# OettlM/STEDM

Measured on AMD Instinct MI355X. Metric: U-Net denoising steps/sec (32x32x4 latent, bs=64), higher is better.
Workload: dtype f16; 1 GPU; HER2-style DDIM-50 + CFG 1.5 (rescale 0.7) denoising step, NS32 U-Net (234.6M params, random-init PRNG weights), 32x32x4 latents + 3-ch layout concat, style vector 512; batch_per_gpu=64, global_batch=64, latent=32x32x4, cfg=cond+uncond per step, parallelism=dp1 (independent latents, no in-loop collective)

## Files before the change

### include/stedm_hip.h

```cpp
#ifndef STEDM_HIP_H
#define STEDM_HIP_H

#include <stdint.h>

#ifdef __cplusplus
extern "C" {
#endif

#define STEDM_ABI_VERSION 31

#define STEDM_F16 0
#define STEDM_BF16 1

#define STEDM_CONV_S1 0
#define STEDM_CONV_DOWN 1
#define STEDM_CONV_UP 2
#define STEDM_CONV_UP_SUBPIXEL 3
#define STEDM_CONV_S2D 4

int stedm_abi_version(void);
const char* stedm_last_error(void);
int stedm_device_cus(void);

#define STEDM_F16G_RAW 1
// ... 106 lines not shown
  float qkv_qscale;
  const float* ln_gamma;
  const float* ln_beta;
  const float* ln_res;
  float ln_eps;
  int32_t out16_stride;
  void* gn_coop;
  const uint32_t* gn_coop_epoch;
  uint32_t* gn_coop_tmo;
  int32_t src16_cstride;
  int32_t k_chan0;
  int32_t w_cin;
  int32_t res_bmod;
  const float* res2;
  int32_t ws_bmod;
} stedm_conv_args;
int stedm_conv_igemm(const stedm_conv_args* args, void* stream);
int stedm_conv_fused_skip_ok(const stedm_conv_args* args);
int stedm_conv3x3_tiles_ok(int Hout, int Wout);
int stedm_im2col_rows16(const void* src16, void* dst16, int B, int Hs, int Ws, int C, int mode, void* stream);
int stedm_conv_rs_ok(const stedm_conv_args* args);
int stedm_conv_partials(const stedm_conv_args* args, int32_t* nshare, int dry, void* stream);
int stedm_conv_finish(const stedm_conv_args* args, int nshare, void* stream);

int stedm_conv_in(const float* x1, int c1, const float* x2, int c2, int x2_bmod, const float* w_oihw,
                  const float* bias, float* out, int B, int H, int W, int cout, float* chan_stats, void* stream);
int stedm_conv_out(const float* src, int c, const float* chan_stats, int nslab, const float* gamma, const float* beta,
                   float eps, int groups, const float* w_hwio, const float* bias, float* out, int B, int H, int W,
                   int cout, void* stream);

// ... 226 lines not shown

int stedm_image_to_uint8(const float* x, unsigned char* out, int B, int C, int H, int W, void* stream);
int stedm_seg_merge(const float* seg, float* out, int B, int K, int H, int W, void* stream);
int stedm_argmax_u8(const float* seg, unsigned char* out, long N, int ncls, void* stream);

int stedm_unfold_tiles(const float* x, float* tiles, int B, int C, int H, int W, int kh, int kw, int sy, int sx, int l0, int nl, void* stream);
int stedm_fold_blend(const float* tiles, const float* w_tile, const float* w_tie, float* out, unsigned char* out_u8, int B, int C, int th, int tw,
                     int sy, int sx, int Ly, int Lx, void* stream);

int stedm_graph_begin(void* stream);
int stedm_graph_end(void* stream, void** graph_exec_out);
int stedm_graph_launch(void* graph_exec, void* stream);
int stedm_graph_destroy(void* graph_exec);

int stedm_debug_conv_stamps(unsigned long long* host_out, int nblocks);

#ifdef __cplusplus
}
#endif
#endif
```

### stedm_amd/_lib.py

```python
from __future__ import annotations

import ctypes as C
import os

_HERE = os.path.dirname(os.path.abspath(__file__))
LIB_PATH = os.environ.get("STEDM_HIP_LIB") or os.path.join(_HERE, "libstedm_hip.so")

ABI_VERSION = 31
F16, BF16 = 0, 1
CONV_S1, CONV_DOWN, CONV_UP, CONV_UP_SUBPIXEL, CONV_S2D = 0, 1, 2, 3, 4
STREAM_POSTERIOR = 0x40000


class StedmHipError(RuntimeError):
    pass


class ConvArgs(C.Structure):
    _fields_ = [
        ("src1", C.c_void_p), ("src2", C.c_void_p),
        ("c1", C.c_int32), ("c2", C.c_int32), ("src2_bmod", C.c_int32),
        ("B", C.c_int32), ("Hin", C.c_int32), ("Win", C.c_int32),
        ("mode", C.c_int32), ("ks", C.c_int32),
        ("scale", C.c_void_p), ("shift", C.c_void_p),
# ... 3 lines not shown
        ("res", C.c_void_p), ("out", C.c_void_p),
        ("cout", C.c_int32), ("npass", C.c_int32), ("mm_dtype", C.c_int32),
        ("src16_hi", C.c_void_p), ("src16_lo", C.c_void_p),
        ("act_out", C.c_int32), ("out16_hi", C.c_void_p), ("out16_lo", C.c_void_p),
        ("w_frag", C.c_void_p), ("chan_stats", C.c_void_p),
        ("src16b_hi", C.c_void_p), ("w_frag_b", C.c_void_p), ("bias_b", C.c_void_p), ("cb", C.c_int32),
        ("ws", C.c_void_p), ("ws_floats", C.c_int64), ("chan_nslab", C.c_int32), ("w_frag16", C.c_void_p), ("w_frag_b16", C.c_void_p), ("pad_br", C.c_int32),
        ("gn_gamma", C.c_void_p), ("gn_beta", C.c_void_p), ("gn_eps", C.c_float), ("gn_groups", C.c_int32), ("gn_act", C.c_int32), ("gn_out16", C.c_void_p), ("gn_mr", C.c_void_p), ("gn_only", C.c_int32),
        ("gn_out16_lo", C.c_void_p),
        ("qkv_q", C.c_void_p), ("qkv_k", C.c_void_p), ("qkv_vt", C.c_void_p),
        ("qkv_T", C.c_int32), ("qkv_Tp", C.c_int32), ("qkv_heads", C.c_int32), ("qkv_qscale", C.c_float),
        ("ln_gamma", C.c_void_p), ("ln_beta", C.c_void_p), ("ln_res", C.c_void_p), ("ln_eps", C.c_float),
        ("out16_stride", C.c_int32),
        ("gn_coop", C.c_void_p), ("gn_coop_epoch", C.c_void_p), ("gn_coop_tmo", C.c_void_p),
        ("src16_cstride", C.c_int32), ("k_chan0", C.c_int32), ("w_cin", C.c_int32), ("res_bmod", C.c_int32),
        ("res2", C.c_void_p), ("ws_bmod", C.c_int32),
    ]


_P, _I, _F = C.c_void_p, C.c_int, C.c_float
SIGNATURES = {
    "stedm_abi_version": (_I, []),
    "stedm_last_error": (C.c_char_p, []),
    "stedm_device_cus": (_I, []),
    "stedm_f16_guard_set": (_I, [_P]),
    "stedm_pack_conv_weight": (_I, [_P, _P, _P, _I, _I, _I, _I, _P]),
    "stedm_pack_conv_weight_up": (_I, [_P, _P, _P, _I, _I, _I, _P]),
    "stedm_pack_conv_weight_frag": (_I, [_P, _P, _I, _I, _I, _I, _P]),
    "stedm_pack_conv_weight_up_frag": (_I, [_P, _P, _I, _I, _I, _P]),
    "stedm_pack_conv_weight_frag16": (_I, [_P, C.c_long, C.c_long, _I, _P, _I, _I, _I, _I, _P]),
    "stedm_pack_conv_weight_frag16_hl": (_I, [_P, C.c_long, C.c_long, _I, _P, _I, _I, _I, _P]),
# ... 137 lines not shown
    "stedm_vq_nearest": (_I, [_P, _P, _I, _I, _I, C.c_long, _P, _P, _P]),
    "stedm_ddim_quantize_x0": (_I, [_P, _P, _P, _P, _P, _P, _I, _I, _I, C.c_long, _P, _P, _P]),
    "stedm_conv1x1_nchw": (_I, [_P, _P, _P, _P, _I, _I, _I, C.c_long, _P]),
    "stedm_softmax_rows16": (_I, [_P, C.c_long, _F, _P, _P, C.c_long, _I, C.c_long, _I, _P]),
    "stedm_gauss_sample": (_I, [_P, _P, _P, _I, _I, C.c_long, _F, _I, C.c_long, C.c_ulonglong, _P]),
    "stedm_image_to_uint8": (_I, [_P, _P, _I, _I, _I, _I, _P]),
    "stedm_seg_merge": (_I, [_P, _P, _I, _I, _I, _I, _P]),
    "stedm_argmax_u8": (_I, [_P, _P, C.c_long, _I, _P]),
    "stedm_unfold_tiles": (_I, [_P, _P, _I, _I, _I, _I, _I, _I, _I, _I, _I, _I, _P]),
    "stedm_fold_blend": (_I, [_P, _P, _P, _P, _P, _I, _I, _I, _I, _I, _I, _I, _I, _P]),
    "stedm_graph_begin": (_I, [_P]),
    "stedm_graph_end": (_I, [_P, C.POINTER(C.c_void_p)]),
    "stedm_graph_launch": (_I, [_P, _P]),
    "stedm_graph_destroy": (_I, [_P]),
    "stedm_debug_conv_stamps": (_I, [_P, _I]),
}

_lib = None


def lib() -> C.CDLL:
    global _lib
    if _lib is None:
        if not os.path.exists(LIB_PATH):
            raise StedmHipError(
                f"{LIB_PATH} not found: build it with `python -m stedm_amd.build` "
                "(there is no CPU / PyTorch fallback for the hot path)")
        try:
            import torch
        except ImportError:
# ... 24 lines not shown
```

### stedm_amd/csrc/conv_common.hpp

```cpp
#pragma once
#include "common.hpp"

typedef float f32x16 __attribute__((ext_vector_type(16)));
typedef float f32x4 __attribute__((ext_vector_type(4)));
typedef _Float16 f16x8 __attribute__((ext_vector_type(8)));
typedef __bf16 bf16x8 __attribute__((ext_vector_type(8)));
typedef _Float16 f16x4 __attribute__((ext_vector_type(4)));
typedef __bf16 bf16x4 __attribute__((ext_vector_type(4)));

constexpr int BN = 128;

struct ConvParams {
  stedm_conv_args a;
  int M, Hout, Wout, HWout, Cin, taps;
  int cstride, w_cin;
  int whole, nsamp, trows;
  int wsplit;
  int PRs, PW, NP;
  int tiles_m, tiles_n;
  unsigned mg_hw, mg_w, mg_pw, mg_prpw;
  int ksplit;
  int stats_done;
  int gn_done;
  int gn_tile;
  int gn_coop;
  int xcd_m;
  int partials;
  int nshare;
  int npers;
  unsigned* ovf;
  int dbg;
};

#ifdef STEDM_CONV_DIAG
#define STEDM_DBG(WORD, BITS) (((WORD) & (BITS)) != 0)
#else
#define STEDM_DBG(WORD, BITS) (0)
#endif

template <typename T>
struct MM;
template <>
struct MM<_Float16> {
  using V8 = f16x8;
  using V4 = f16x4;
  static __device__ __forceinline__ f32x16 mfma(V8 a, V8 b, f32x16 c) {
    return __builtin_amdgcn_mfma_f32_32x32x16_f16(a, b, c, 0, 0, 0);
  }
  static __device__ __forceinline__ f32x4 mfma16(V8 a, V8 b, f32x4 c) {
    return __builtin_amdgcn_mfma_f32_16x16x32_f16(a, b, c, 0, 0, 0);
  }
};
template <>
// ... 3 lines not shown
  static __device__ __forceinline__ f32x16 mfma(V8 a, V8 b, f32x16 c) {
    return __builtin_amdgcn_mfma_f32_32x32x16_bf16(a, b, c, 0, 0, 0);
  }
  static __device__ __forceinline__ f32x4 mfma16(V8 a, V8 b, f32x4 c) {
    return __builtin_amdgcn_mfma_f32_16x16x32_bf16(a, b, c, 0, 0, 0);
  }
};


#define STEDM_ZERO_PAGE_BYTES 135168

namespace stedm {
bool conv_geometry(ConvParams& p, int bm, bool allow_wsplit = false);
int conv_launch_dma(ConvParams& p, hipStream_t st, bool dry = false);
int conv_splitk_finish(ConvParams& p, int nshare, hipStream_t st);
}
```

### stedm_amd/csrc/conv_dma_bf16_p1.hip

```cpp
#include "conv_igemm_dma9.inc"
#include "conv_rs.inc"
namespace stedm {
int conv_dma_pick_bf16_p1(ConvParams& p, hipStream_t st, bool dry) {
  int rc = conv_rs_pick<__bf16>(p, st, dry);
  if (rc >= 0 || dry || p.a.src16b_hi || p.a.mode == STEDM_CONV_S2D || p.a.qkv_q || p.a.ln_gamma) return rc;
  if (p.a.src16_cstride || p.a.k_chan0 || p.a.w_cin || p.a.res_bmod || p.a.res2 || p.partials || p.a.out16_stride) return rc;
  rc = dma9_pick<__bf16>(p, st);
  return rc >= 0 ? rc : dma_pick<1, __bf16>(p, st);
}
}

extern "C" int stedm_debug_conv_stamps(unsigned long long* host_out, int nblocks) {
  if (!host_out || nblocks <= 0 || nblocks > 2048) { stedm::set_error("debug_conv_stamps: bad args"); return 1; }
  hipError_t e = hipMemcpyFromSymbol(host_out, HIP_SYMBOL(g_conv_stamps), (size_t)nblocks * 8 * sizeof(unsigned long long));
  if (e != hipSuccess) { stedm::set_error("debug_conv_stamps: %s", hipGetErrorString(e)); return 2; }
  return 0;
}
```

### stedm_amd/csrc/conv_igemm_dma.hip

```cpp
#include "conv_common.hpp"
using namespace stedm;

namespace stedm {
int conv_dma_pick_f16_p1(ConvParams&, hipStream_t, bool dry);
int conv_dma_pick_f16_p3(ConvParams&, hipStream_t, bool dry);
int conv_dma_pick_bf16_p1(ConvParams&, hipStream_t, bool dry);
int conv_dma_pick_bf16_p3(ConvParams&, hipStream_t, bool dry);
}

int stedm::conv_launch_dma(ConvParams& p, hipStream_t st, bool dry) {
  const stedm_conv_args& a = p.a;
  if (a.src16b_hi && a.npass != 1) { set_error("conv_igemm(dma): the fused skip phase is single-product only"); return 1; }
  if (dry && a.npass != 1 && !a.w_frag16) return 1;
  if (a.src16b_hi && ((long)a.B * a.Hin * a.Win * a.cb >= (1L << 31) || a.cb * 2 + 256 > STEDM_ZERO_PAGE_BYTES)) {
    set_error("conv_igemm(dma): fused skip operand too large (cb=%d)", a.cb);
    return 1;
  }
  if ((long)a.B * a.Hin * a.Win * (p.cstride > p.Cin ? p.cstride : p.Cin) >= (1L << 31)) {
    set_error("conv_igemm(dma): activation tensor too large for 32-bit element offsets");
    return 1;
  }
  if (p.Cin * 2 + 256 > STEDM_ZERO_PAGE_BYTES) { set_error("conv_igemm(dma): Cin too large for the zero page"); return 1; }
  const bool f16 = a.mm_dtype == STEDM_F16;
  int rc = a.npass == 3 ? (f16 ? conv_dma_pick_f16_p3(p, st, dry) : conv_dma_pick_bf16_p3(p, st, dry))
// ... 13 lines not shown
```

### stedm_amd/csrc/conv_rs.inc

```
#pragma once
#include <type_traits>

#include "conv_igemm_dma.inc"
#include "gn_fold.hpp"

static __device__ unsigned long long g_conv_stamps[2048 * 8];
#define STAMP(K) if (STEDM_DBG(p.dbg, 1024) && tid == 0 && blockIdx.x < 2048) g_conv_stamps[blockIdx.x * 8 + (K)] = wall_clock64()
#define STAMPC(K) if (STEDM_DBG(p.dbg, 1024) && tid == 0 && blockIdx.x < 2048) g_conv_stamps[blockIdx.x * 8 + (K)] = __builtin_amdgcn_s_memtime()

#ifdef STEDM_CONV_DIAG
#define RS_DIAG(BIT) ((STEDM_CONV_DIAG) & (BIT))
#else
#define RS_DIAG(BIT) 0
#endif

__device__ __forceinline__ float rs_lane_xor1(float v) {
  return __builtin_bit_cast(float, __builtin_amdgcn_mov_dpp(__builtin_bit_cast(int, v), 0xB1, 0xF, 0xF, true));
}
template <typename T>
__device__ __forceinline__ unsigned rs_pack2(float lo, float hi) {
  typedef T V2T __attribute__((ext_vector_type(2)));
  V2T v; v[0] = (T)lo; v[1] = (T)hi;
  return __builtin_bit_cast(unsigned, v);
}
// ... 28 lines not shown
    GLDB(bf[ST][0], sb_, 0); GLDB(bf[ST][1], sb_, 1024);                       \
  }
#define LOAD_A(BASE, SUB, ST)                                                  \
  {                                                                            \
    const unsigned pb_ = (BASE) + ((SUB) / NTAB) * a_plane;                    \
    _Pragma("unroll") for (int i_ = 0; i_ < WM; ++i_) { const unsigned a_ = pb_ + aofs[(SUB) % NTAB][i_]; LDSR(af[ST][i_], a_); } \
  }
#define LOAD_A1(BASE, SUB, ST, I)                                              \
  {                                                                            \
    const unsigned a_ = (BASE) + ((SUB) / NTAB) * a_plane + aofs[(SUB) % NTAB][I]; \
    LDSR(af[ST][I], a_);                                                       \
  }
#pragma unroll
  for (int k = 0; k < NSB; ++k) LOAD_B(k, k)
  if (FIRST) __syncthreads();
  {
    const unsigned Afirst = A0 + abuf * a_buf;
#pragma unroll
    for (int k = 0; k < LA; ++k) LOAD_A(Afirst, k, k)
  }
  if constexpr (!SPREAD) {
  for (int step = 0; step < nchunks; ++step) {
    const unsigned Acur = A0 + abuf * a_buf;
    if (++abuf == NABUF) abuf = 0;
    const unsigned Anext = step + 1 < nchunks ? A0 + abuf * a_buf : Acur;
    const int g0 = step * NS;
#pragma unroll
    for (int t = 0; t < NS; ++t) {
      if (!NOBAR && t == NS - LA - 1) __builtin_amdgcn_s_barrier();
      __builtin_amdgcn_sched_barrier(0);
#pragma unroll
      for (int j = 0; j < 2; ++j) acc[0][j] = RS_MFMA(af[t % NSA][0], bf[t % NSB][j], acc[0][j]);
      __builtin_amdgcn_sched_barrier(0);
      if (t + LA < NS) LOAD_A(Acur, t + LA, (t + LA) % NSA) else LOAD_A(Anext, t + LA - NS, (t + LA) % NSA)
      __builtin_amdgcn_sched_barrier(0);
// ... 62 lines not shown
    wcur = wsb + ((size_t)(unsigned)g_ << 13);                                 \
  }
#define W_LOAD(ST, C) if constexpr (!RS_DIAG(16)) bf[ST][C] = *reinterpret_cast<const V8*>(wcur + (C) * 1024);
#define A_ADDR(DST, BASE, TAP, HF, I)                                                                         \
  {                                                                                                           \
    if constexpr (NSETS == 1) asm volatile("v_add_u32 %0, %1, %2" : "=v"(DST) : "s"((BASE) + tapd[TAP]), "v"(aofs[0][(HF) * 4 + (I)])); \
    else asm volatile("v_add_u32 %0, %1, %2" : "=v"(DST) : "s"(BASE), "v"(aofs[NSETS == 1 ? 0 : (TAP)][(HF) * 4 + (I)]));           \
  }
#pragma unroll
  for (int k = 0; k < NSB; ++k) {
    W_ADDR(k)
#pragma unroll
    for (int c = 0; c < 4; ++c) W_LOAD(k, c)
  }
  if (FIRST) __syncthreads();
  {
    const unsigned Afirst = A0 + abuf * a_buf;
#pragma unroll
    for (int i = 0; i < 4; ++i) { unsigned a_; A_ADDR(a_, Afirst, 0, 0, i) if constexpr (!RS_DIAG(8)) LDSR(af[i], a_); }
  }
  for (int step = 0; step < nchunks; ++step) {
    const unsigned Acur = A0 + abuf * a_buf;
    if (++abuf == NABUF) abuf = 0;
    const unsigned Anext = step + 1 < nchunks ? A0 + abuf * a_buf : Acur;
    const int g0 = step * NS;
#pragma unroll
    for (int u = 0; u < NU; ++u) {
      const int t = u >> 1, hf = u & 1;
      if (u == NU - 1 && !RS_DIAG(32)) __builtin_amdgcn_s_barrier();
#pragma unroll
      for (int i = 0; i < 4; ++i) {
        const int pi = (i + 3) & 3;
        const int tu = i == 0 ? u : u + 1;
        unsigned a_ = 0;
#pragma unroll
// ... 178 lines not shown
    tile_n = (j - jm * tn_x) * gn + x / gm;
    tile_m = jm * gm + x % gm;
  }
  constexpr bool npers = NPERS;
  if (npers) { tile_m = bid / p.npers; tile_n = (bid % p.npers) * (p.tiles_n / p.npers); }
  if STEDM_DBG(p.dbg, 256) { tile_n = 0; tile_m = 0; }
  const int m0 = tile_m * BMT, n0 = tile_n * BN;
  const int nchunks_all = p.Cin / BKC;
  const int nchunks_w = p.w_cin / BKC;
  const int nsteps = split ? nchunks_all / p.ksplit : nchunks_all;
  const int cbeg = kz * nsteps;
  const int nsteps2_all = FUSE ? a.cb / 64 : 0;
  const int nsteps2 = split ? nsteps2_all / p.ksplit : nsteps2_all;
  const int c2beg = split ? kz * nsteps2 : 0;
  STAMP(0);

  int b0, yo0;
  if (p.whole) { b0 = tile_m * p.nsamp; yo0 = 0; }
  else { b0 = m0 / p.HWout; yo0 = (m0 - b0 * p.HWout) / p.Wout; }
  const int br = s2d ? a.pad_br : 0;
  const int x0 = p.wsplit ? (m0 - b0 * p.HWout) - yo0 * p.Wout : 0;
  const int srow0 = ((a.mode == STEDM_CONV_S1 || SUBPIX) ? yo0 - 1 : (yo0 - 1) >> 1) + br;
  static_assert(RS_3X3 == 0, "");

  auto div_hw = [&](int n) { return (int)__umulhi((unsigned)n, p.mg_hw); };
  auto div_w = [&](int n) { return (int)__umulhi((unsigned)n, p.mg_w); };
  auto div_pw = [&](int n) { return (int)__umulhi((unsigned)n, p.mg_pw); };
  auto div_prpw = [&](int n) { return (int)__umulhi((unsigned)n, p.mg_prpw); };
  const int rem0 = GEO1 ? m0 - (m0 / p.HWout) * p.HWout : 0;
  auto patch_pixel = [&](int pos) {
    int off = -1;
    if (pos < p.NP) {
      if (GEO1) { if (m0 + pos < p.M) off = m0 + pos; }
      else {
        const int s_ = div_prpw(pos), rem = pos - s_ * (p.PRs * p.PW);
        const int prow = div_pw(rem), pcol = rem - prow * p.PW;
        const int b = b0 + s_, sy = srow0 + prow, sx = x0 + pcol - 1 + br;
        if (b < a.B && sy >= 0 && sy < a.Hin && sx >= 0 && sx < a.Win) off = (b * a.Hin + sy) * a.Win + sx;
      }
    }
    return off;
  };
  constexpr int NTC = NCW * 64;
  if (!is_loader) {
  for (int ml = tid; ml < BMT; ml += NTC) {
    int s_ = 0, yl = 0, x = 0, y = 0;
    if (!GEO1) {
      if (p.whole) { s_ = div_hw(ml); const int rem = ml - s_ * p.HWout; yl = div_w(rem); x = rem - yl * p.Wout; y = yl; }
      else { yl = div_w(ml); x = ml - yl * p.Wout; y = yo0 + yl; }
    }
#pragma unroll
    for (int tap = 0; tap < (M16 ? 1 : TAPS); ++tap) {
      int pos;
      if (GEO1) pos = ml;
      else {
        const int dy = SUBPIX ? (tap >> 1) + py : tap / 3, dx = SUBPIX ? (tap & 1) + px : tap - (tap / 3) * 3;
        int prow, pcol;
        if (a.mode == STEDM_CONV_S1 || SUBPIX) { prow = yl + dy; pcol = x + dx; }
        else { prow = ((y + dy - 1) >> 1) - srow0; pcol = ((x + dx - 1) >> 1) + 1; }
        pos = (s_ * p.PRs + prow) * p.PW + pcol;
      }
      sIdx[tap * BMT + ml] = (pos * BROW) | (M16 ? 0 : ((((pos / RPB) % CPP) ^ (IS1X1 ? 2 * tap : 0)) << 24));
    }
  }
  for (int ml = tid; ml < BMT; ml += NTC) {
    int m, b;
    if (GEO1) { m = m0 + ml; b = (IS1X1 && a.qkv_q) ? m / a.qkv_T : m0 / p.HWout + div_hw(rem0 + ml); }
    else if (!p.whole) { m = m0 + ml; b = b0; }
    else { const int s_ = div_hw(ml); b = b0 + s_; m = b * p.HWout + (ml - s_ * p.HWout); }
    const bool okm = m < p.M;
    if (SUBPIX && !s2d && okm) {
      const int rem = m - b * p.HWout, y = div_w(rem), x = rem - y * p.Wout;
      m = (b * 2 * p.Hout + 2 * y + py) * (2 * p.Wout) + 2 * x + px;
    }
    sM[ml] = okm ? m : -1;
    sMb[ml] = b;
  }
// ... 15 lines not shown
    for (int k = 0; k < MAXS; ++k) {
      asrc[k] = zero16;
      if (k < nslots) {
        const int pos = (aw + 2 * k) * PPI + lpos;
        const int logical = M16 ? lphys : lphys ^ ((pos / RPB) % CPP);
        const int pix = patch_pixel(pos);
        asrc[k] = (pix >= 0 ? a_hi + (long)pix * p.cstride : zero16) + logical * 8;
        if (P3 && pix < 0) zmask |= 1u << k;
        if (!STEDM_DBG(p.dbg, 2)) {
#pragma unroll
          for (int pl = 0; pl < NPL; ++pl) {
            GLDS16(asrc[k] + (cbeg * NPL + pl) * (BROW / 2), sA + pl * (a_plane + pl_skew) + (aw + 2 * k) * 1024);
            if (P3) GLDS16(LO_SRC(k) + (cbeg * NPL + pl) * (BROW / 2), sA + a_half + pl * (a_plane + pl_skew) + (aw + 2 * k) * 1024);
          }
        }
      }
    }
    auto issue_a = [&](int chunk) {
      if STEDM_DBG(p.dbg, 2) return;
      unsigned char* dsta = sA + (chunk % NABUF) * a_buf;
#pragma unroll
      for (int pl = 0; pl < NPL; ++pl) {
        const int c0 = ((cbeg + chunk) * NPL + pl) * (BROW / 2);
#pragma unroll
        for (int k = 0; k < MAXS; ++k) {
          if (k < nslots) {
            GLDS16(asrc[k] + c0, dsta + pl * (a_plane + pl_skew) + (aw + 2 * k) * 1024);
            if (P3) GLDS16(LO_SRC(k) + c0, dsta + a_half + pl * (a_plane + pl_skew) + (aw + 2 * k) * 1024);
          }
        }
      }
    };
    if constexpr (P3) {
      if (nsteps > 1) issue_a(1);
      __syncthreads();
      WAIT_VM(0);
      __syncthreads();
      for (int s = 0; s < nsteps; ++s) {
        WAIT_VM(0);
        __builtin_amdgcn_s_barrier();
        if (s + 2 < nsteps) issue_a(s + 2);
      }
    } else {
    early[0] = true;
#pragma unroll
    for (int c = 1; c < 3; ++c)
      if (c < nsteps) { issue_a(c); early[c] = true; }
    __syncthreads();
    int aoff2[FUSE ? 16 : 1];
    if (FUSE) {
#pragma unroll
      for (int k = 0; k < 16; ++k) {
        const int ml = (aw + 2 * k) * 8 + (lane >> 3);
        const int logical = (lane & 7) ^ ((ml >> 1) & 7);
        const int m = sM[ml];
        aoff2[k] = m >= 0 ? m * a.cb + logical * 8 : -(logical * 8) - 1;
      }
    }
    auto issue2 = [&](int c2, int ringpos) {
      if STEDM_DBG(p.dbg, 2) return;
      const uint16_t* b_hi = reinterpret_cast<const uint16_t*>(a.src16b_hi);
      unsigned char* dsta = sA + ringpos * a_buf;
      const int c0 = (c2beg + c2) * 64;
#pragma unroll
      for (int k = 0; k < (FUSE ? 16 : 0); ++k) {
        const int o = aoff2[k];
        const uint16_t* sh = o >= 0 ? b_hi + o + c0 : zero16 + (-o - 1) + c0;
        GLDS16(sh, dsta + (aw + 2 * k) * 1024);
      }
    };
    auto issue_any = [&](int chunk) {
      if (!FUSE || chunk < nsteps) issue_a(chunk); else issue2(chunk - nsteps, chunk % NABUF);
    };
    const int ntot = nsteps + nsteps2;
    auto wait_keep = [&](int cnt) {
      switch (cnt) {
        case 1: WAIT_VM(1); break; case 2: WAIT_VM(2); break; case 3: WAIT_VM(3); break; case 4: WAIT_VM(4); break;
        case 5: WAIT_VM(5); break; case 6: WAIT_VM(6); break; case 7: WAIT_VM(7); break; case 8: WAIT_VM(8); break;
        case 9: WAIT_VM(9); break; case 10: WAIT_VM(10); break; case 11: WAIT_VM(11); break; case 12: WAIT_VM(12); break;
        case 13: WAIT_VM(13); break; case 14: WAIT_VM(14); break; case 15: WAIT_VM(15); break; case 16: WAIT_VM(16); break;
        case 18: WAIT_VM(18); break; case 20: WAIT_VM(20); break; case 22: WAIT_VM(22); break; case 24: WAIT_VM(24); break;
        default: WAIT_VM(0); break;
      }
    };
    auto wait_all_but = [&](int chunk) { wait_keep((FUSE && chunk >= nsteps) ? 16 : nslots * NPL); };
    {
      if (!early[0]) issue_any(0);
      if (ntot > 1 && !early[1]) issue_any(1);
      if (ntot > 2 && !early[2]) issue_any(2);
      if (ntot > 2 && !STEDM_DBG(p.dbg, 2)) wait_all_but(2); else WAIT_VM(0);
      __syncthreads();
      for (int s = 0; s < ntot; ++s) {
        if STEDM_DBG(p.dbg, 4) { if (s + 1 >= ntot) WAIT_VM(0); }
        else if (s + 2 < ntot && !STEDM_DBG(p.dbg, 2)) wait_all_but(s + 2); else WAIT_VM(0);
        if (!(M16 && RS_DIAG(32))) __builtin_amdgcn_s_barrier();
        if (s + 3 < ntot) issue_any(s + 3);
      }
    }
    }
    if (npers) return;
#undef LO_SRC
#undef WAIT_VM
  } else {
    __syncthreads();
    STAMP(1);
    STAMPC(2);
    const int wm = wave >> 1, wn = wave & 1;
    const int r = lane & 31, h = lane >> 5;
    const unsigned voff = lane * 16;
    int abuf = 0;
    const unsigned A0 = (unsigned)(uintptr_t)sA;
    if constexpr (M16) {
      const int r16 = lane & 15;
      unsigned aofs[1][8];
#pragma unroll
      for (int f = 0; f < 8; ++f) {
        const int e = sIdx[wm * 128 + f * 16 + r16];
        if (G1) aofs[0][f] = (unsigned)(e & 0xFFFFFF) + (unsigned)(lane >> 4) * 16u;
        else aofs[0][f] = (unsigned)(e & 0xFFFFFF) + (unsigned)h * 16u + (unsigned)((lane >> 4) & 1) * (unsigned)(a_plane + pl_skew);
      }
      unsigned tapd[NS];
#pragma unroll
      for (int t = 0; t < NS; ++t)
        tapd[t] = G1 ? 0u : (SUBM ? (unsigned)((t >> 1) * p.PW + (t & 1)) * 32u : (unsigned)((t / 3) * p.PW + (t % 3)) * 32u);
      const unsigned char* wq = reinterpret_cast<const unsigned char*>(a.w_frag16) +
                                (((((size_t)parity * p.tiles_n + tile_n) * nchunks_w + cbeg) * NS) * 8 + wn * 4) * 1024;
      f32x4 acc[8][4];
#pragma unroll
      for (int i = 0; i < 8; ++i)
#pragma unroll
        for (int j = 0; j < 4; ++j)
#pragma unroll
          for (int e = 0; e < 4; ++e) acc[i][j][e] = 0.f;
      if constexpr (P3) {
        const size_t wlo = (size_t)((SUBPIX && !s2d) ? 4 : 1) * p.tiles_n * nchunks_all * NS * 8 * 1024;
// ... 17 lines not shown
      STAMP(3);
      STAMPC(7);
      if (!STEDM_DBG(p.dbg, 64)) {
        const int g4 = lane >> 4;
#pragma unroll
        for (int i = 0; i < 8; ++i)
#pragma unroll
          for (int j = 0; j < 4; ++j) {
            float* dst = sStage + (wm * 128 + i * 16 + g4 * 4) * SST + wn * 64 + j * 16 + r16;
#pragma unroll
            for (int e = 0; e < 4; ++e) dst[e * SST] = acc[i][j][e];
          }
      }
    } else {
    unsigned aofs[TAPS][WM];
#pragma unroll
    for (int t = 0; t < TAPS; ++t)
#pragma unroll
      for (int i = 0; i < WM; ++i) {
        const int e = sIdx[t * BMT + wm * (WM * 32) + i * 32 + r];
        aofs[t][i] = (unsigned)(e & 0xFFFFFF) + ((((unsigned)e >> 24) ^ (unsigned)h) << 4);
      }
    const unsigned char* wq = reinterpret_cast<const unsigned char*>(a.w_frag) +
                              ((((size_t)parity * p.tiles_n + tile_n) * nchunks_w + cbeg) * NS * 4 + wn * 2) * 1024;

    f32x16 acc[WM][2];
    if constexpr (NPERS) {
      {
        const unsigned N = (unsigned)a.cout;
        const int HD = a.qkv_heads * 64, Tn = a.qkv_T;
        const unsigned Tp = (unsigned)a.qkv_Tp;
        const unsigned esz = a.out ? 4u : 2u;
        const unsigned out_bytes = STEDM_DBG(p.dbg, 2048) ? 0u : (unsigned)p.M * N * esz;
        const unsigned pl_bytes = (a.qkv_q && !STEDM_DBG(p.dbg, 2048)) ? (unsigned)(p.M / Tn) * (unsigned)HD * Tp * 2u : 0u;
        const auto rs_out = __builtin_amdgcn_make_buffer_rsrc(a.out ? (void*)a.out : a.out16_hi, 0, out_bytes, 0x00020000);
        const auto rs_res = __builtin_amdgcn_make_buffer_rsrc((void*)a.res, 0, a.res ? out_bytes : 0u, 0x00020000);
        const auto rs_q = __builtin_amdgcn_make_buffer_rsrc(a.qkv_q, 0, pl_bytes, 0x00020000);
// ... 817 lines not shown
    const int nt = p.HWout / BMT;
    static const bool off = getenv("STEDM_NO_GN_COOP") != nullptr;
    if (!p.gn_tile && !off && cpg > 0 && stats && q.ksplit < 2 && (KIND == RS_3X3 || KIND == RS_3X3M) && !FUSE && !P3 && p.HWout % BMT == 0 && nt >= 2 && nt <= 4 &&
        a_.cout == 128 && p.tiles_n == 1 && p.xcd_m == 0 && !p.whole && cpg % 4 == 0 && 128 % cpg == 0 && 256 % a_.gn_groups == 0 && a_.out && !a_.out16_hi && !a_.act_out &&
        a_.gn_coop && a_.gn_coop_epoch && a_.gn_coop_tmo && (size_t)lds + 4 * 128 * 2 * sizeof(float) <= LDS_MAX)
      p.gn_coop = nt;
  }
  p.npers = 0;
  if (KIND == RS_1X1N) {
    const long cus = stedm_device_cus() > 0 ? stedm_device_cus() : 256;
    auto cost = [&](int s_) { return ((long)p.tiles_m * s_ + cus - 1) / cus * (2 + p.tiles_n / s_); };
    p.npers = (p.tiles_n % 2 == 0 && p.tiles_n >= 4 && cost(2) < cost(1)) ? 2 : 1;
  }
  ConvParams kp = p;
  if (!stats) kp.a.chan_stats = nullptr;
  if (q.a.k_chan0) {
    kp.a.src16_hi = reinterpret_cast<const unsigned char*>(q.a.src16_hi) + (size_t)q.a.k_chan0 * 2;
    if (q.a.w_frag) kp.a.w_frag = reinterpret_cast<const unsigned char*>(q.a.w_frag) + (size_t)q.a.k_chan0 * 9 * 256;
    if (q.a.w_frag16) kp.a.w_frag16 = reinterpret_cast<const unsigned char*>(q.a.w_frag16) + (size_t)q.a.k_chan0 * 9 * 256;
  }
  auto k = conv_rs_kernel<T, WM, KIND, FUSE, P3>;
  const size_t lds_launch = lds + (p.gn_coop ? (size_t)4 * 128 * 2 * sizeof(float) : 0);
  static size_t lds_set = 0;
  if (lds_launch > lds_set) {
    hipError_t e = hipFuncSetAttribute(reinterpret_cast<const void*>(k), hipFuncAttributeMaxDynamicSharedMemorySize, (int)lds_launch);
    if (e != hipSuccess) { set_error("conv_igemm(rs): hipFuncSetAttribute(%zu) failed: %s", lds_launch, hipGetErrorString(e)); return 2; }
    lds_set = lds_launch;
  }
  if (kp.ksplit >= 2) kp.a.chan_stats = nullptr;
  k<<<p.npers ? p.tiles_m * p.npers : p.tiles_m * p.tiles_n * ((SUBK && !s2d) ? 4 : 1) * (kp.ksplit >= 2 ? kp.ksplit : 1), (16 / WM + 2) * 64, lds_launch, st>>>(kp);
// ... 109 lines not shown
```

### stedm_amd/ops.py

```python
from __future__ import annotations

import ctypes as C
from dataclasses import dataclass
from typing import Optional, Tuple

import torch

from . import _lib
from ._lib import BF16, CONV_DOWN, CONV_S1, CONV_S2D, CONV_UP, CONV_UP_SUBPIXEL, F16, STREAM_POSTERIOR, ConvArgs, check, lib


@dataclass(frozen=True)
class Precision:
    mm_dtype: int = F16
    npass: int = 3
    attn_fp8: bool = False

    @staticmethod
    def parse(name: str) -> "Precision":
        table = {"parity": Precision(F16, 3), "parity_bf16": Precision(BF16, 3),
                 "fast": Precision(F16, 1), "f16": Precision(F16, 1), "bf16": Precision(BF16, 1),
                 "fp8": Precision(BF16, 1, True), "bf16+fp8attn": Precision(BF16, 1, True)}
        if name not in table:
            raise ValueError(f"unknown precision {name!r}; choose from {sorted(table)}")
# ... 441 lines not shown
    return conv_igemm(None, w_hi.view(cout, 1, 9 * C), None if w_lo is None else w_lo.view(cout, 1, 9 * C), out, prec=prec, ks=1, mode=CONV_S1,
                      src16=(cols[0], cols[1]), **kw)


def conv_igemm(src1: Optional[torch.Tensor], w_hi: torch.Tensor, w_lo: Optional[torch.Tensor], out: torch.Tensor, *, prec: Precision,
               ks: int = 3, mode: int = CONV_S1, src2: Optional[torch.Tensor] = None, src2_bmod: int = 0,
               scale: Optional[torch.Tensor] = None, shift: Optional[torch.Tensor] = None, act: int = 0,
               bias: Optional[torch.Tensor] = None, emb: Optional[torch.Tensor] = None, emb_offset: int = 0,
               emb_bstride: int = 0, res: Optional[torch.Tensor] = None,
               src16: Optional[Tuple[torch.Tensor, Optional[torch.Tensor]]] = None, act_out: int = 0,
               out16: Optional[Tuple[torch.Tensor, Optional[torch.Tensor]]] = None, w_frag: Optional[torch.Tensor] = None,
               chan_stats: Optional[torch.Tensor] = None,
               skip: Optional[Tuple[torch.Tensor, torch.Tensor, Optional[torch.Tensor]]] = None, query_fused: bool = False, query_rs: bool = False,
               ws: Optional[torch.Tensor] = None, pad_br: bool = False, w_frag16: Optional[torch.Tensor] = None,
               gn_next: Optional[tuple] = None, qkv_planes: Optional[tuple] = None, ln_after: Optional[tuple] = None, coop: Optional[tuple] = None,
               out16_stride: int = 0, cout: Optional[int] = None, res_bmod: int = 0, res2: Optional[torch.Tensor] = None, partials: bool = False):
    if src16 is not None and src1 is None and ks == 3 and mode in (CONV_S1, CONV_DOWN, CONV_UP) and not out16_stride:
        _, H_, W_, _ = src16[0].shape
        Ho_, Wo_ = ((H_ - 1) // 2 + 1, (W_ - 1) // 2 + 1) if mode == CONV_DOWN else ((2 * H_, 2 * W_) if mode == CONV_UP else (H_, W_))
        if not conv3x3_tiles_ok(Ho_, Wo_):
            if query_fused or query_rs:
                return False
            if not src16[0].is_contiguous() or res_bmod or res2 is not None or partials:
                raise _lib.StedmHipError("conv_igemm: a K window / res_bmod belongs to the tiled register-streamed kernel; this output grid takes the im2col form")
            return _conv3x3_generic(src16, w_hi, w_lo, out, prec=prec, mode=mode, scale=scale, shift=shift, act=act, bias=bias, emb=emb,
                                    emb_offset=emb_offset, emb_bstride=emb_bstride, res=res, act_out=act_out, out16=out16, chan_stats=chan_stats,
                                    skip=skip, ws=ws, gn_next=gn_next)
    if out is not None:
        _chk(out, name="out")
    a = ConvArgs()
    a.act_out = act_out
# ... 83 lines not shown
            base = s16._base if s16._base is not None else s16
            k0 = (s16.storage_offset() - base.storage_offset()) % cs
            assert src1 is None and tuple(s16.stride()) == (Hin * Win * cs, Win * cs, cs, 1) and k0 + c1 <= cs, \
                "src16[0] must be contiguous or a view plane[b0:b1, :, :, k0:k1] of a contiguous plane"
            assert cs % 32 == 0 and k0 % 32 == 0 and c1 % 32 == 0, "a K window is cut on 32-channel boundaries"
            kwin = True
            a.src16_hi = s16.data_ptr() - 2 * k0
            if a.src16_lo is not None:
                assert tuple(src16[1].stride()) == tuple(s16.stride()) and src16[1].storage_offset() == s16.storage_offset()
                a.src16_lo = src16[1].data_ptr() - 2 * k0
            a.src16_cstride, a.k_chan0 = cs, k0
            wplanes = w_hi._val[0] if isinstance(w_hi, LazyPlanes) and w_hi._val is not None else (None if isinstance(w_hi, LazyPlanes) else w_hi)
            a.w_cin = (w_frag.shape[-5] * 16 if w_frag is not None and prec.npass == 1 else
                       w_frag16.shape[-5] * 32 if w_frag16 is not None else wplanes.shape[-1] if wplanes is not None else cs)
            assert w_frag is None or w_frag16 is None or w_frag.shape[-5] * 16 == w_frag16.shape[-5] * 32
    a.res_bmod = int(res_bmod)
    if res_bmod:
        assert res is not None and res.is_contiguous() and res.dtype == torch.float32 and B % res_bmod == 0 and res.shape[0] >= res_bmod
    if res2 is not None:
        assert res is not None and res2.is_contiguous() and res2.dtype == torch.float32 and tuple(res2.shape) == tuple(res.shape)
        a.res2 = res2.data_ptr()
    a.c1, a.c2, a.src2_bmod = c1, c2, src2_bmod
    a.B, a.Hin, a.Win = B, Hin, Win
    a.mode, a.ks = mode, ks
    a.scale, a.shift, a.act = _ptr(scale), _ptr(shift), act
    lazy = w_hi if isinstance(w_hi, LazyPlanes) else None
    if lazy is not None:
        w_hi, w_lo = lazy._val if lazy._val is not None else (w_frag if w_frag is not None else w_frag16, None)
    a.w_hi, a.w_lo = _ptr(w_hi), (_ptr(w_lo) if prec.npass == 3 else None)
    a.bias = _ptr(bias)
# ... 1327 lines not shown
```

Before: 172.0 steps/s.

## Precompute conv gather-offset tables in global memory to shorten kernel prologue

For stride-1 3x3 and subpixel register-streamed convs, the per-geometry A-gather offset table is now built once on the host, cached in device memory and keyed by geometry. Kernels read it straight from global memory instead of rebuilding it in LDS each launch, which also lets them skip a prologue __syncthreads when the table is present. The loader prologue is reworked as well: one fewer early chunk is issued, the wait and barrier order changes, and the wait-count switch is extended. Prologue timestamp probes are added for debugging. The table is built lazily and is skipped during graph capture, so the first uncaptured call adds an allocation.

Result: no change. 172.9 steps/s (median of 6 runs) (+0.5%).

```diff
diff --git a/include/stedm_hip.h b/include/stedm_hip.h
--- a/include/stedm_hip.h
+++ b/include/stedm_hip.h
@@ -144,6 +144,7 @@
   int32_t res_bmod;
   const float* res2;
   int32_t ws_bmod;
+  int32_t geo_tables_off;
 } stedm_conv_args;
 int stedm_conv_igemm(const stedm_conv_args* args, void* stream);
 int stedm_conv_fused_skip_ok(const stedm_conv_args* args);
@@ -400,6 +401,9 @@
 int stedm_graph_destroy(void* graph_exec);
 
 int stedm_debug_conv_stamps(unsigned long long* host_out, int nblocks);
+int stedm_debug_conv_prologue_stamps(unsigned long long* host_out, int nblocks);
+int stedm_conv_gather_table_host(int32_t* out, int m16, int subpix, int npar, int whole, int HWout, int Wout, int PRs, int PW);
+int stedm_conv_gather_table_count(void);
 
 #ifdef __cplusplus
 }
diff --git a/stedm_amd/_lib.py b/stedm_amd/_lib.py
--- a/stedm_amd/_lib.py
+++ b/stedm_amd/_lib.py
@@ -41,7 +41,7 @@
         ("out16_stride", C.c_int32),
         ("gn_coop", C.c_void_p), ("gn_coop_epoch", C.c_void_p), ("gn_coop_tmo", C.c_void_p),
         ("src16_cstride", C.c_int32), ("k_chan0", C.c_int32), ("w_cin", C.c_int32), ("res_bmod", C.c_int32),
-        ("res2", C.c_void_p), ("ws_bmod", C.c_int32),
+        ("res2", C.c_void_p), ("ws_bmod", C.c_int32), ("geo_tables_off", C.c_int32),
     ]
 
 
@@ -209,6 +209,9 @@
     "stedm_graph_launch": (_I, [_P, _P]),
     "stedm_graph_destroy": (_I, [_P]),
     "stedm_debug_conv_stamps": (_I, [_P, _I]),
+    "stedm_debug_conv_prologue_stamps": (_I, [_P, _I]),
+    "stedm_conv_gather_table_host": (_I, [_P, _I, _I, _I, _I, _I, _I, _I, _I]),
+    "stedm_conv_gather_table_count": (_I, []),
 }
 
 _lib = None
diff --git a/stedm_amd/csrc/conv_common.hpp b/stedm_amd/csrc/conv_common.hpp
--- a/stedm_amd/csrc/conv_common.hpp
+++ b/stedm_amd/csrc/conv_common.hpp
@@ -28,6 +28,7 @@
   int partials;
   int nshare;
   int npers;
+  const int* geo_tab;
   unsigned* ovf;
   int dbg;
 };
@@ -37,6 +38,32 @@
 #else
 #define STEDM_DBG(WORD, BITS) (0)
 #endif
+
+struct RsTabGeo {
+  int whole, HWout, Wout, PRs, PW;
+  unsigned mg_hw, mg_w;
+};
+__host__ __device__ __forceinline__ unsigned rs_magic(int d) { return (unsigned)((0x100000000ull + (unsigned)d - 1) / (unsigned)d); }
+__host__ __device__ __forceinline__ int rs_mulhi(int n, unsigned mg) {
+#ifdef __HIP_DEVICE_COMPILE__
+  return (int)__umulhi((unsigned)n, mg);
+#else
+  return (int)(((unsigned long long)(unsigned)n * mg) >> 32);
+#endif
+}
+__host__ __device__ __forceinline__ void rs_tile_row(const RsTabGeo& g, int ml, int& s_, int& yl, int& x) {
+  if (g.whole) { s_ = rs_mulhi(ml, g.mg_hw); const int rem = ml - s_ * g.HWout; yl = rs_mulhi(rem, g.mg_w); x = rem - yl * g.Wout; }
+  else { s_ = 0; yl = rs_mulhi(ml, g.mg_w); x = ml - yl * g.Wout; }
+}
+__host__ __device__ __forceinline__ int rs_tap_pos(const RsTabGeo& g, int s_, int yl, int x, int dy, int dx) { return (s_ * g.PRs + yl + dy) * g.PW + x + dx; }
+__host__ __device__ __forceinline__ int rs_tab_word32(int pos, bool m16) { return (pos * 32) | (m16 ? 0 : (((pos / 8) % 2) << 24)); }
+__host__ __device__ __forceinline__ int rs_tab_rows(bool m16, bool subpix) { return m16 ? 1 : (subpix ? 4 : 9); }
+__host__ __device__ __forceinline__ int rs_tab_entry(const RsTabGeo& g, bool m16, bool subpix, int par, int tap, int ml) {
+  int s_, yl, x;
+  rs_tile_row(g, ml, s_, yl, x);
+  const int dy = subpix ? (tap >> 1) + (par >> 1) : tap / 3, dx = subpix ? (tap & 1) + (par & 1) : tap - (tap / 3) * 3;
+  return rs_tab_word32(rs_tap_pos(g, s_, yl, x, dy, dx), m16);
+}
 
 template <typename T>
 struct MM;
@@ -70,4 +97,5 @@
 bool conv_geometry(ConvParams& p, int bm, bool allow_wsplit = false);
 int conv_launch_dma(ConvParams& p, hipStream_t st, bool dry = false);
 int conv_splitk_finish(ConvParams& p, int nshare, hipStream_t st);
+const int* conv_gather_table(const ConvParams& p, bool m16, bool subpix, int npar, hipStream_t st);
 }
diff --git a/stedm_amd/csrc/conv_dma_bf16_p1.hip b/stedm_amd/csrc/conv_dma_bf16_p1.hip
--- a/stedm_amd/csrc/conv_dma_bf16_p1.hip
+++ b/stedm_amd/csrc/conv_dma_bf16_p1.hip
@@ -16,3 +16,9 @@
   if (e != hipSuccess) { stedm::set_error("debug_conv_stamps: %s", hipGetErrorString(e)); return 2; }
   return 0;
 }
+extern "C" int stedm_debug_conv_prologue_stamps(unsigned long long* host_out, int nblocks) {
+  if (!host_out || nblocks <= 0 || nblocks > 2048) { stedm::set_error("debug_conv_prologue_stamps: bad args"); return 1; }
+  hipError_t e = hipMemcpyFromSymbol(host_out, HIP_SYMBOL(g_conv_pro), (size_t)nblocks * 8 * sizeof(unsigned long long));
+  if (e != hipSuccess) { stedm::set_error("debug_conv_prologue_stamps: %s", hipGetErrorString(e)); return 2; }
+  return 0;
+}
diff --git a/stedm_amd/csrc/conv_igemm_dma.hip b/stedm_amd/csrc/conv_igemm_dma.hip
--- a/stedm_amd/csrc/conv_igemm_dma.hip
+++ b/stedm_amd/csrc/conv_igemm_dma.hip
@@ -1,3 +1,7 @@
+#include <map>
+#include <mutex>
+#include <vector>
+
 #include "conv_common.hpp"
 using namespace stedm;
 
@@ -6,6 +10,61 @@
 int conv_dma_pick_f16_p3(ConvParams&, hipStream_t, bool dry);
 int conv_dma_pick_bf16_p1(ConvParams&, hipStream_t, bool dry);
 int conv_dma_pick_bf16_p3(ConvParams&, hipStream_t, bool dry);
+}
+
+namespace {
+struct GeoKey {
+  int dev, m16, subpix, npar, whole, HWout, Wout, PRs, PW;
+  bool operator<(const GeoKey& o) const { return memcmp(this, &o, sizeof(GeoKey)) < 0; }
+};
+std::mutex g_geo_mu;
+std::map<GeoKey, const int*> g_geo_tabs;
+
+int gather_table_fill(int* out, int m16, int subpix, int npar, int whole, int HWout, int Wout, int PRs, int PW) {
+  const RsTabGeo g{whole, HWout, Wout, PRs, PW, rs_magic(HWout), rs_magic(Wout)};
+  const int rows = rs_tab_rows(m16 != 0, subpix != 0);
+  int n = 0;
+  for (int par = 0; par < npar; ++par)
+    for (int tap = 0; tap < rows; ++tap)
+      for (int ml = 0; ml < 256; ++ml) out[n++] = rs_tab_entry(g, m16 != 0, subpix != 0, par, tap, ml);
+  return n;
+}
+}
+
+const int* stedm::conv_gather_table(const ConvParams& p, bool m16, bool subpix, int npar, hipStream_t st) {
+  GeoKey k;
+  memset(&k, 0, sizeof(k));
+  if (hipGetDevice(&k.dev) != hipSuccess) return nullptr;
+  k.m16 = m16; k.subpix = subpix; k.npar = npar; k.whole = p.whole; k.HWout = p.HWout; k.Wout = p.Wout; k.PRs = p.PRs; k.PW = p.PW;
+  std::lock_guard<std::mutex> lock(g_geo_mu);
+  auto it = g_geo_tabs.find(k);
+  if (it != g_geo_tabs.end()) return it->second;
+  hipStreamCaptureStatus cs = hipStreamCaptureStatusNone;
+  if (hipStreamIsCapturing(st, &cs) != hipSuccess || cs != hipStreamCaptureStatusNone) return nullptr;
+  std::vector<int> host((size_t)npar * rs_tab_rows(m16, subpix) * 256);
+  gather_table_fill(host.data(), m16, subpix, npar, k.whole, k.HWout, k.Wout, k.PRs, k.PW);
+  int* dev = nullptr;
+  if (hipMalloc(&dev, host.size() * sizeof(int)) != hipSuccess) { (void)hipGetLastError(); return nullptr; }
+  if (hipMemcpy(dev, host.data(), host.size() * sizeof(int), hipMemcpyHostToDevice) != hipSuccess) { (void)hipGetLastError(); (void)hipFree(dev); return nullptr; }
+  g_geo_tabs.emplace(k, dev);
+  return dev;
+}
+
+extern "C" int stedm_conv_gather_table_host(int32_t* out, int m16, int subpix, int npar, int whole, int HWout, int Wout, int PRs, int PW) {
+  if (!out || (npar != 1 && npar != 4) || HWout <= 0 || Wout <= 0 || HWout % Wout != 0 || PRs <= 0 || PW <= 0 || (long)PRs * PW >= 65536 ||
+      (long)HWout * Wout >= (1l << 32) || (whole && 256 % HWout != 0)) {
+    set_error("conv_gather_table_host: bad geometry");
+    return -1;
+  }
+  return gather_table_fill(out, m16, subpix, npar, whole, HWout, Wout, PRs, PW);
+}
+
+extern "C" int stedm_conv_gather_table_count(void) {
+  int dev = 0, n = 0;
+  if (hipGetDevice(&dev) != hipSuccess) { (void)hipGetLastError(); return 0; }
+  std::lock_guard<std::mutex> lock(g_geo_mu);
+  for (const auto& kv : g_geo_tabs) n += kv.first.dev == dev;
+  return n;
 }
 
 int stedm::conv_launch_dma(ConvParams& p, hipStream_t st, bool dry) {
diff --git a/stedm_amd/csrc/conv_rs.inc b/stedm_amd/csrc/conv_rs.inc
--- a/stedm_amd/csrc/conv_rs.inc
+++ b/stedm_amd/csrc/conv_rs.inc
@@ -7,6 +7,11 @@
 static __device__ unsigned long long g_conv_stamps[2048 * 8];
 #define STAMP(K) if (STEDM_DBG(p.dbg, 1024) && tid == 0 && blockIdx.x < 2048) g_conv_stamps[blockIdx.x * 8 + (K)] = wall_clock64()
 #define STAMPC(K) if (STEDM_DBG(p.dbg, 1024) && tid == 0 && blockIdx.x < 2048) g_conv_stamps[blockIdx.x * 8 + (K)] = __builtin_amdgcn_s_memtime()
+
+static __device__ unsigned long long g_conv_pro[2048 * 8];
+#define STAMPP_(DBG, K) if (STEDM_DBG(DBG, 1024) && threadIdx.x == 0 && blockIdx.x < 2048) g_conv_pro[blockIdx.x * 8 + (K)] = wall_clock64()
+#define STAMPP(K) STAMPP_(p.dbg, K)
+#define STAMPL(K) if (STEDM_DBG(p.dbg, 1024) && tid == NCW * 64 && blockIdx.x < 2048) g_conv_pro[blockIdx.x * 8 + (K)] = wall_clock64()
 
 #ifdef STEDM_CONV_DIAG
 #define RS_DIAG(BIT) ((STEDM_CONV_DIAG) & (BIT))
@@ -66,11 +71,13 @@
 #pragma unroll
   for (int k = 0; k < NSB; ++k) LOAD_B(k, k)
   if (FIRST) __syncthreads();
+  if (FIRST) STAMPP_(dbg, 2);
   {
     const unsigned Afirst = A0 + abuf * a_buf;
 #pragma unroll
     for (int k = 0; k < LA; ++k) LOAD_A(Afirst, k, k)
   }
+  if (FIRST) STAMPP_(dbg, 3);
   if constexpr (!SPREAD) {
   for (int step = 0; step < nchunks; ++step) {
     const unsigned Acur = A0 + abuf * a_buf;
@@ -163,11 +170,13 @@
     for (int c = 0; c < 4; ++c) W_LOAD(k, c)
   }
   if (FIRST) __syncthreads();
+  if (FIRST) STAMPP_(dbg, 2);
   {
     const unsigned Afirst = A0 + abuf * a_buf;
 #pragma unroll
     for (int i = 0; i < 4; ++i) { unsigned a_; A_ADDR(a_, Afirst, 0, 0, i) if constexpr (!RS_DIAG(8)) LDSR(af[i], a_); }
   }
+  if (FIRST) STAMPP_(dbg, 3);
   for (int step = 0; step < nchunks; ++step) {
     const unsigned Acur = A0 + abuf * a_buf;
     if (++abuf == NABUF) abuf = 0;
@@ -376,6 +385,7 @@
   const int nsteps2 = split ? nsteps2_all / p.ksplit : nsteps2_all;
   const int c2beg = split ? kz * nsteps2 : 0;
   STAMP(0);
+  STAMPP(0);
 
   int b0, yo0;
   if (p.whole) { b0 = tile_m * p.nsamp; yo0 = 0; }
@@ -404,25 +414,25 @@
     return off;
   };
   constexpr int NTC = NCW * 64;
+  constexpr bool TABK = (IS3X3 || SUBPIX) && !P3;
+  const bool tabs = TABK && p.geo_tab != nullptr;
+  const RsTabGeo tg{p.whole, p.HWout, p.Wout, p.PRs, p.PW, p.mg_hw, p.mg_w};
   if (!is_loader) {
+  if (!tabs)
   for (int ml = tid; ml < BMT; ml += NTC) {
     int s_ = 0, yl = 0, x = 0, y = 0;
-    if (!GEO1) {
-      if (p.whole) { s_ = div_hw(ml); const int rem = ml - s_ * p.HWout; yl = div_w(rem); x = rem - yl * p.Wout; y = yl; }
-      else { yl = div_w(ml); x = ml - yl * p.Wout; y = yo0 + yl; }
-    }
+    if (!GEO1) { rs_tile_row(tg, ml, s_, yl, x); y = p.whole ? yl : yo0 + yl; }
 #pragma unroll
     for (int tap = 0; tap < (M16 ? 1 : TAPS); ++tap) {
       int pos;
       if (GEO1) pos = ml;
       else {
         const int dy = SUBPIX ? (tap >> 1) + py : tap / 3, dx = SUBPIX ? (tap & 1) + px : tap - (tap / 3) * 3;
-        int prow, pcol;
-        if (a.mode == STEDM_CONV_S1 || SUBPIX) { prow = yl + dy; pcol = x + dx; }
-        else { prow = ((y + dy - 1) >> 1) - srow0; pcol = ((x + dx - 1) >> 1) + 1; }
-        pos = (s_ * p.PRs + prow) * p.PW + pcol;
-      }
-      sIdx[tap * BMT + ml] = (pos * BROW) | (M16 ? 0 : ((((pos / RPB) % CPP) ^ (IS1X1 ? 2 * tap : 0)) << 24));
+        if (a.mode == STEDM_CONV_S1 || SUBPIX) pos = rs_tap_pos(tg, s_, yl, x, dy, dx);
+        else { const int prow = ((y + dy - 1) >> 1) - srow0, pcol = ((x + dx - 1) >> 1) + 1; pos = (s_ * p.PRs + prow) * p.PW + pcol; }
+      }
+      if (BROW == 32) sIdx[tap * BMT + ml] = rs_tab_word32(pos, M16);
+      else sIdx[tap * BMT + ml] = (pos * BROW) | (M16 ? 0 : ((((pos / RPB) % CPP) ^ (IS1X1 ? 2 * tap : 0)) << 24));
     }
   }
   for (int ml = tid; ml < BMT; ml += NTC) {
@@ -468,8 +478,10 @@
             if (P3) GLDS16(LO_SRC(k) + (cbeg * NPL + pl) * (BROW / 2), sA + a_half + pl * (a_plane + pl_skew) + (aw + 2 * k) * 1024);
           }
         }
-      }
-    }
+        if (k == 0) STAMPL(4);
+      }
+    }
+    STAMPL(5);
     auto issue_a = [&](int chunk) {
       if STEDM_DBG(p.dbg, 2) return;
       unsigned char* dsta = sA + (chunk % NABUF) * a_buf;
@@ -498,16 +510,17 @@
     } else {
     early[0] = true;
 #pragma unroll
-    for (int c = 1; c < 3; ++c)
+    for (int c = 1; c < 2; ++c)
       if (c < nsteps) { issue_a(c); early[c] = true; }
-    __syncthreads();
+    STAMPL(6);
+    if (!tabs) __syncthreads();
     int aoff2[FUSE ? 16 : 1];
     if (FUSE) {
 #pragma unroll
       for (int k = 0; k < 16; ++k) {
         const int ml = (aw + 2 * k) * 8 + (lane >> 3);
         const int logical = (lane & 7) ^ ((ml >> 1) & 7);
-        const int m = sM[ml];
+        const int m = tabs ? (m0 + ml < p.M ? m0 + ml : -1) : sM[ml];
         aoff2[k] = m >= 0 ? m * a.cb + logical * 8 : -(logical * 8) - 1;
       }
     }
@@ -528,22 +541,29 @@
     };
     const int ntot = nsteps + nsteps2;
     auto wait_keep = [&](int cnt) {
+      if (cnt > 16) cnt = cnt > 52 ? 52 : cnt & ~1;
       switch (cnt) {
         case 1: WAIT_VM(1); break; case 2: WAIT_VM(2); break; case 3: WAIT_VM(3); break; case 4: WAIT_VM(4); break;
         case 5: WAIT_VM(5); break; case 6: WAIT_VM(6); break; case 7: WAIT_VM(7); break; case 8: WAIT_VM(8); break;
         case 9: WAIT_VM(9); break; case 10: WAIT_VM(10); break; case 11: WAIT_VM(11); break; case 12: WAIT_VM(12); break;
         case 13: WAIT_VM(13); break; case 14: WAIT_VM(14); break; case 15: WAIT_VM(15); break; case 16: WAIT_VM(16); break;
         case 18: WAIT_VM(18); break; case 20: WAIT_VM(20); break; case 22: WAIT_VM(22); break; case 24: WAIT_VM(24); break;
+        case 26: WAIT_VM(26); break; case 28: WAIT_VM(28); break; case 30: WAIT_VM(30); break; case 32: WAIT_VM(32); break;
+        case 34: WAIT_VM(34); break; case 36: WAIT_VM(36); break; case 38: WAIT_VM(38); break; case 40: WAIT_VM(40); break;
+        case 42: WAIT_VM(42); break; case 44: WAIT_VM(44); break; case 46: WAIT_VM(46); break; case 48: WAIT_VM(48); break;
+        case 50: WAIT_VM(50); break; case 52: WAIT_VM(52); break;
         default: WAIT_VM(0); break;
       }
     };
-    auto wait_all_but = [&](int chunk) { wait_keep((FUSE && chunk >= nsteps) ? 16 : nslots * NPL); };
+    auto chunk_cnt = [&](int chunk) { return chunk >= ntot ? 0 : ((FUSE && chunk >= nsteps) ? 16 : nslots * NPL); };
+    auto wait_all_but = [&](int chunk) { wait_keep(chunk_cnt(chunk)); };
     {
       if (!early[0]) issue_any(0);
       if (ntot > 1 && !early[1]) issue_any(1);
+      if (!STEDM_DBG(p.dbg, 2)) wait_keep(chunk_cnt(1)); else WAIT_VM(0);
+      STAMPL(7);
+      __syncthreads();
       if (ntot > 2 && !early[2]) issue_any(2);
-      if (ntot > 2 && !STEDM_DBG(p.dbg, 2)) wait_all_but(2); else WAIT_VM(0);
-      __syncthreads();
       for (int s = 0; s < ntot; ++s) {
         if STEDM_DBG(p.dbg, 4) { if (s + 1 >= ntot) WAIT_VM(0); }
         else if (s + 2 < ntot && !STEDM_DBG(p.dbg, 2)) wait_all_but(s + 2); else WAIT_VM(0);
@@ -556,23 +576,29 @@
 #undef LO_SRC
 #undef WAIT_VM
   } else {
-    __syncthreads();
+    if (!tabs) __syncthreads();
     STAMP(1);
     STAMPC(2);
+    STAMPP(1);
     const int wm = wave >> 1, wn = wave & 1;
     const int r = lane & 31, h = lane >> 5;
     const unsigned voff = lane * 16;
     int abuf = 0;
     const unsigned A0 = (unsigned)(uintptr_t)sA;
+    const int __attribute__((address_space(1)))* gtab = reinterpret_cast<const int __attribute__((address_space(1)))*>((uintptr_t)p.geo_tab);
+    const int __attribute__((address_space(3)))* lidx = reinterpret_cast<const int __attribute__((address_space(3)))*>((unsigned)(uintptr_t)sIdx);
     if constexpr (M16) {
       const int r16 = lane & 15;
       unsigned aofs[1][8];
-#pragma unroll
-      for (int f = 0; f < 8; ++f) {
-        const int e = sIdx[wm * 128 + f * 16 + r16];
-        if (G1) aofs[0][f] = (unsigned)(e & 0xFFFFFF) + (unsigned)(lane >> 4) * 16u;
-        else aofs[0][f] = (unsigned)(e & 0xFFFFFF) + (unsigned)h * 16u + (unsigned)((lane >> 4) & 1) * (unsigned)(a_plane + pl_skew);
-      }
+      auto fill16 = [&](auto tab) {
+#pragma unroll
+        for (int f = 0; f < 8; ++f) {
+          const int e = tab[wm * 128 + f * 16 + r16];
+          if (G1) aofs[0][f] = (unsigned)(e & 0xFFFFFF) + (unsigned)(lane >> 4) * 16u;
+          else aofs[0][f] = (unsigned)(e & 0xFFFFFF) + (unsigned)h * 16u + (unsigned)((lane >> 4) & 1) * (unsigned)(a_plane + pl_skew);
+        }
+      };
+      if (tabs) fill16(gtab + parity * BMT); else fill16(lidx);
       unsigned tapd[NS];
 #pragma unroll
       for (int t = 0; t < NS; ++t)
@@ -620,13 +646,16 @@
       }
     } else {
     unsigned aofs[TAPS][WM];
-#pragma unroll
-    for (int t = 0; t < TAPS; ++t)
-#pragma unroll
-      for (int i = 0; i < WM; ++i) {
-        const int e = sIdx[t * BMT + wm * (WM * 32) + i * 32 + r];
-        aofs[t][i] = (unsigned)(e & 0xFFFFFF) + ((((unsigned)e >> 24) ^ (unsigned)h) << 4);
-      }
+    auto fill = [&](auto tab) {
+#pragma unroll
+      for (int t = 0; t < TAPS; ++t)
+#pragma unroll
+        for (int i = 0; i < WM; ++i) {
+          const int e = tab[t * BMT + wm * (WM * 32) + i * 32 + r];
+          aofs[t][i] = (unsigned)(e & 0xFFFFFF) + ((((unsigned)e >> 24) ^ (unsigned)h) << 4);
+        }
+    };
+    if (tabs) fill(gtab + parity * TAPS * BMT); else fill(lidx);
     const unsigned char* wq = reinterpret_cast<const unsigned char*>(a.w_frag) +
                               ((((size_t)parity * p.tiles_n + tile_n) * nchunks_w + cbeg) * NS * 4 + wn * 2) * 1024;
 
@@ -1474,6 +1503,10 @@
   }
   ConvParams kp = p;
   if (!stats) kp.a.chan_stats = nullptr;
+  kp.geo_tab = nullptr;
+  if constexpr ((KIND == RS_3X3 || KIND == RS_3X3M || SUBK) && !P3) {
+    if (!q.a.geo_tables_off && (SUBK || q.a.mode == STEDM_CONV_S1)) kp.geo_tab = conv_gather_table(p, M16, SUBK, (SUBK && !s2d) ? 4 : 1, st);
+  }
   if (q.a.k_chan0) {
     kp.a.src16_hi = reinterpret_cast<const unsigned char*>(q.a.src16_hi) + (size_t)q.a.k_chan0 * 2;
     if (q.a.w_frag) kp.a.w_frag = reinterpret_cast<const unsigned char*>(q.a.w_frag) + (size_t)q.a.k_chan0 * 9 * 256;
diff --git a/stedm_amd/ops.py b/stedm_amd/ops.py
--- a/stedm_amd/ops.py
+++ b/stedm_amd/ops.py
@@ -479,7 +479,8 @@
                skip: Optional[Tuple[torch.Tensor, torch.Tensor, Optional[torch.Tensor]]] = None, query_fused: bool = False, query_rs: bool = False,
                ws: Optional[torch.Tensor] = None, pad_br: bool = False, w_frag16: Optional[torch.Tensor] = None,
                gn_next: Optional[tuple] = None, qkv_planes: Optional[tuple] = None, ln_after: Optional[tuple] = None, coop: Optional[tuple] = None,
-               out16_stride: int = 0, cout: Optional[int] = None, res_bmod: int = 0, res2: Optional[torch.Tensor] = None, partials: bool = False):
+               out16_stride: int = 0, cout: Optional[int] = None, res_bmod: int = 0, res2: Optional[torch.Tensor] = None, partials: bool = False,
+               geo_tables: bool = True):
     if src16 is not None and src1 is None and ks == 3 and mode in (CONV_S1, CONV_DOWN, CONV_UP) and not out16_stride:
         _, H_, W_, _ = src16[0].shape
         Ho_, Wo_ = ((H_ - 1) // 2 + 1, (W_ - 1) // 2 + 1) if mode == CONV_DOWN else ((2 * H_, 2 * W_) if mode == CONV_UP else (H_, W_))
@@ -593,6 +594,7 @@
             a.w_cin = (w_frag.shape[-5] * 16 if w_frag is not None and prec.npass == 1 else
                        w_frag16.shape[-5] * 32 if w_frag16 is not None else wplanes.shape[-1] if wplanes is not None else cs)
             assert w_frag is None or w_frag16 is None or w_frag.shape[-5] * 16 == w_frag16.shape[-5] * 32
+    a.geo_tables_off = 0 if geo_tables else 1
     a.res_bmod = int(res_bmod)
     if res_bmod:
         assert res is not None and res.is_contiguous() and res.dtype == torch.float32 and B % res_bmod == 0 and res.shape[0] >= res_bmod
```
